# JunzheJosephZhu/DenseMatcher

Measured on AMD Instinct MI355X. Metric: mesh-pairs/sec at N=2048 D=768 k=128, higher is better.
Workload: dtype f16; 1 GPU; configs[1]: batch=64 pairs, N=2048, D=768, k=128 functional-map solve; pairs_per_gpu=64, N=2048, D=768, k=128, basis_dtype=float64, parallelism=pairs sharded over 1 GPU(s), one process per GPU, no data-path collective, process_group_size=1

## Files before the change

densematcher_amd/csrc/dm_exact.h:

```cpp
#pragma once
#include "dm_device.h"
#include "dm_internal.h"

struct ks_exact_args {
    const double* AT; const double* BT; const double* n1; const double* massS; const double* massT;
    int K, N2, N2pad, N1, N1pad, Kpad;
    dm_simnn_queue q;
    int32_t* nn;
    const void* Trow = nullptr; const void* Crow = nullptr; int ldrow = 0; int ldcrow = 0;
};

template <int KIND, typename TR, typename TC>
__device__ __forceinline__ void ks_exact_row(const ks_exact_args& a, int o, float thr, double* xrow, unsigned long long* cmask) {
    const double* __restrict__ AT = a.AT; const double* __restrict__ BT = a.BT; const double* __restrict__ n1 = a.n1;
    const double* __restrict__ massS = a.massS; const double* __restrict__ massT = a.massT;
    const int K = a.K, N2 = a.N2, N2pad = a.N2pad, N1 = a.N1, N1pad = a.N1pad, Kpad = a.Kpad;
    const float* __restrict__ qpb = a.q.pb; const int32_t* __restrict__ qpj = a.q.pj; const float* __restrict__ qps = a.q.ps;
    const int nparts = a.q.nparts, pw = a.q.pw, Npad_s = a.q.Npad, nsub = nparts * (pw / 32);
    int32_t* __restrict__ nn = a.nn;
    double* part_s = xrow + K;
    const TR* __restrict__ Trow = reinterpret_cast<const TR*>(a.Trow);
    const TC* __restrict__ Crow = reinterpret_cast<const TC*>(a.Crow);
    const int ldrow = a.ldrow, ldcrow = a.ldcrow ? a.ldcrow : a.ldrow;
    const int t = threadIdx.x;
    const int c = Crow ? (t >> 3) : (t & 31), part = Crow ? (t & 7) : (t >> 5);
    {
        const int b = o / N2, i = o - b * N2;
        const double* A = AT ? AT + (long long)b * Kpad * N2pad + i : nullptr;
        const double* Bm = BT ? BT + (long long)b * Kpad * N1pad : nullptr;
        auto keep_of = [&](int sbt) -> bool {
            const int q = min((sbt * 32) / pw, nparts - 1);
            const long long oq = ((long long)b * nparts + q) * Npad_s + i;
            const float vs = qps[oq], vb = qpb[oq];
            const int vj = qpj[oq];
            return sbt < nsub && (vs >= thr || (vb >= thr && (vj >> 5) == sbt));
        };
        bool keep = keep_of(t);
        __syncthreads();
        if (Trow) { for (int r = t; r < K; r += 256) xrow[r] = (double)Trow[((long long)b * N2 + i) * ldrow + r]; }
        else { for (int r = t; r < K; r += 256) xrow[r] = A[(long long)r * N2pad]; }
        __syncthreads();
        double bv = KIND == 0 ? DM_INF_F64 : -DM_INF_F64;
        int bj = DM_IDX_NONE;
        const double mt = KIND == 2 ? massT[(long long)b * N2 + i] : 0.0;
        for (int sb0 = 0; sb0 < nsub; sb0 += 256) {
            if (sb0) keep = keep_of(sb0 + t);
            const unsigned long long km = __ballot(keep);
            if ((t & 63) == 0) cmask[t >> 6] = km;
            __syncthreads();
            for (int w = 0; w < 4; ++w) {
                unsigned long long mm = cmask[w];
                while (mm) {
                    const int sb = sb0 + w * 64 + __ffsll((long long)mm) - 1;
                    mm &= mm - 1;
                    const int j = sb * 32 + c;
                    double sacc = 0.0;
                    if (j < N1 && Crow) {
                        const TC* Cr = Crow + ((long long)b * N1 + j) * ldcrow;
                        int r = part;
                        for (; r + 56 < K; r += 64) {
                            TC y[8];
#pragma unroll
                            for (int u = 0; u < 8; ++u) y[u] = Cr[r + 8 * u];
#pragma unroll
                            for (int u = 0; u < 8; ++u) sacc = fma(xrow[r + 8 * u], (double)y[u], sacc);
                        }
                        for (; r < K; r += 8) sacc = fma(xrow[r], (double)Cr[r], sacc);
                    } else if (j < N1) {
                        int r = part;
                        for (; r + 56 < K; r += 64) {
                            double y[8];
#pragma unroll
                            for (int u = 0; u < 8; ++u) y[u] = Bm[(long long)(r + 8 * u) * N1pad + j];
#pragma unroll
                            for (int u = 0; u < 8; ++u) sacc = fma(xrow[r + 8 * u], y[u], sacc);
                        }
                        for (; r < K; r += 8) sacc = fma(xrow[r], Bm[(long long)r * N1pad + j], sacc);
                    }
                    part_s[part * 32 + c] = sacc;
                    __syncthreads();
                    if (t < 32 && sb * 32 + t < N1) {
                        const int j = sb * 32 + t;
                        double g = part_s[t];
#pragma unroll
                        for (int q = 1; q < 8; ++q) g += part_s[q * 32 + t];
                        if (KIND == 0) {
                            const double v = n1[(long long)b * N1pad + j] - 2.0 * g;
                            if (v < bv) { bv = v; bj = j; }
                        } else {
                            const double v = g * (KIND == 1 ? massS[(long long)b * N1 + j] : mt);
                            if (v > bv) { bv = v; bj = j; }
                        }
                    }
                    __syncthreads();
                }
            }
            __syncthreads();
        }
        if (t < 32) {
#pragma unroll
            for (int off = 1; off < 32; off <<= 1) {
                const double ov = __shfl_xor(bv, off);
                const int oj = __shfl_xor(bj, off);
                if (KIND == 0) argmin_merge(bv, bj, ov, oj); else argmax_merge(bv, bj, ov, oj);
            }
            if (t == 0 && bj != DM_IDX_NONE) nn[o] = bj;
        }
    }
}
```

densematcher_amd/csrc/dm_knnsplit.hip:

```cpp
#include "dm_device.h"
#include "dm_internal.h"
#include "dm_split.h"
#include "dm_exact.h"

static inline int pad_to(int x, int m) { return (x + m - 1) / m * m; }

constexpr int KS_NCH = DM_NCH;
constexpr int KS_BIAS = 8;

__global__ __launch_bounds__(256) void ks_absmax_kernel(const double* __restrict__ AT, int K, int N2, int N2pad, int Kpad,
                                                        double* __restrict__ amax) {
    __shared__ double sh[4];
    const int chunk = blockIdx.x, b = blockIdx.y, t = threadIdx.x;
    const double* M = AT + (long long)b * Kpad * N2pad;
    double m = 0.0;
    for (int r = chunk; r < K; r += KS_NCH)
        for (int c = t; c < N2; c += 256) m = fmax(m, fabs(M[(long long)r * N2pad + c]));
#pragma unroll
    for (int off = 32; off > 0; off >>= 1) m = fmax(m, __shfl_xor(m, off));
    if ((t & 63) == 0) sh[t >> 6] = m;
    __syncthreads();
    if (t == 0) amax[b * KS_NCH + chunk] = fmax(fmax(sh[0], sh[1]), fmax(sh[2], sh[3]));
}

struct fs_bias_set {
    const double* nrm; int N, Npad; const double* mass; float* bias; unsigned int* bmax; unsigned int* mmax; float* scale32;
    int rows_out;
    const double* hint; int32_t* force;
    double* pair_out;
};
__device__ __forceinline__ void fs_bias_body(const fs_bias_set& s, int b, int chunk, const double* __restrict__ amaxT, int nT,
                                             const double* __restrict__ amaxS, int nS) {
    __shared__ float wb[4], wm[4];
    const int j = chunk * 256 + threadIdx.x;
    if (chunk * 256 >= s.N) return;
    const double sx_ = ks_scale(amaxT + b * nT, nT);
    const double sxy = sx_ * ks_scale(amaxS + b * nS, nS);
    if (chunk == 0 && threadIdx.x == 0) {
        if (s.hint && ks_scale(s.hint + b, 1) != sx_) s.force[b] = 1;
        if (s.pair_out) { double m_ = 0.0; for (int q = 0; q < nT; ++q) m_ = fmax(m_, amaxT[b * nT + q]); s.pair_out[b] = m_; }
    }
    float bb = 0.f, mm = 0.f;
    if (j < s.N) {
        const float v = (float)(-0.5 * s.nrm[(long long)b * s.Npad + j] * sxy);
        s.bias[(long long)b * s.rows_out + j] = v;
        bb = fabsf(v);
        if (s.mass) {
            const float m32 = (float)s.mass[(long long)b * s.N + j];
            s.scale32[(long long)b * s.rows_out + j] = m32;
            mm = fabsf(m32);
        }
    }
#pragma unroll
    for (int off = 32; off > 0; off >>= 1) { bb = fmaxf(bb, __shfl_xor(bb, off)); mm = fmaxf(mm, __shfl_xor(mm, off)); }
    if ((threadIdx.x & 63) == 0) { wb[threadIdx.x >> 6] = bb; wm[threadIdx.x >> 6] = mm; }
    __syncthreads();
    if (threadIdx.x == 0) {
        bb = fmaxf(fmaxf(wb[0], wb[1]), fmaxf(wb[2], wb[3]));
        mm = fmaxf(fmaxf(wm[0], wm[1]), fmaxf(wm[2], wm[3]));
        atomicMax(s.bmax + b, __float_as_uint(bb));
        if (s.mass) atomicMax(s.mmax + b, __float_as_uint(mm));
    }
}

template <bool SRC>
__global__ __launch_bounds__(256) void ks_build_kernel(const double* __restrict__ M, const double* __restrict__ n1,
                                                       const double* __restrict__ amaxT, const double* __restrict__ amaxS, int nS,
                                                       int K, int N, int Npad, int Kpad, int ld, int fill, int head,
                                                       _Float16* __restrict__ F, int32_t* __restrict__ overflow, int paired, int nT,
                                                       int rows_out,
                                                       int nbuild, fs_bias_set sA, fs_bias_set sB, int nbb) {
    if ((int)blockIdx.x < 2 * nbb) {
        const int e = (int)blockIdx.x;
        fs_bias_body(e < nbb ? sA : sB, blockIdx.y, e < nbb ? e : e - nbb, amaxT, nT, amaxS, nS);
        return;
    }
    (void)nbuild;
    extern __shared__ __attribute__((aligned(16))) _Float16 ks_img[];
    const int ldl = fill + 8;
    const int b = blockIdx.y, v0 = ((int)blockIdx.x - 2 * nbb) * 64;
    const int vl = threadIdx.x & 63, rg = threadIdx.x >> 6;
    const int v = v0 + vl;
    const double sx = ks_scale(amaxT + b * nT, nT);
    const double sc = SRC ? ks_scale(amaxS + b * nS, nS) : sx;
    _Float16* row = ks_img + vl * ldl;
    if (v < N && paired) {
        for (int r0 = rg * 16; r0 < K; r0 += 64) {
            const double* col = M + ((long long)b * Kpad + r0) * Npad + v;
            _Float16* dst = row + 2 * r0;
            f16x8 o[4];
            if (r0 + 16 <= K) {
#pragma unroll
                for (int q = 0; q < 16; ++q) {
                    _Float16 h, l;
                    split2_hw(col[(long long)q * Npad] * sc, h, l);
                    o[q >> 3][q & 7] = h;
                    o[2 + (q >> 3)][q & 7] = l;
                }
            } else {
#pragma unroll
                for (int q = 0; q < 16; ++q) {
                    _Float16 h = (_Float16)0.0f, l = (_Float16)0.0f;
                    if (r0 + q < K) split2_hw(col[(long long)q * Npad] * sc, h, l);
                    o[q >> 3][q & 7] = h;
                    o[2 + (q >> 3)][q & 7] = l;
                }
            }
#pragma unroll
            for (int q = 0; q < 4; ++q) *reinterpret_cast<f16x8*>(dst + 8 * q) = o[q];
        }
    } else if (v < N) {
        for (int r0 = rg * 16; r0 < K; r0 += 64) {
            const double* col = M + ((long long)b * Kpad + r0) * Npad + v;
            _Float16* dst = row + head + 3 * r0;
            if (r0 + 16 <= K) {
                f16x8 o[6];
#pragma unroll
                for (int q = 0; q < 16; ++q) {
                    _Float16 h, l;
                    split2_hw(col[(long long)q * Npad] * sc, h, l);
                    const int e = 3 * q;
                    o[e >> 3][e & 7] = h;
                    o[(e + 1) >> 3][(e + 1) & 7] = SRC ? l : h;
                    o[(e + 2) >> 3][(e + 2) & 7] = SRC ? h : l;
                }
#pragma unroll
                for (int q = 0; q < 6; ++q) *reinterpret_cast<f16x8*>(dst + 8 * q) = o[q];
            } else {
                for (int q = 0; r0 + q < K; ++q) {
                    _Float16 h, l;
                    split2_hw(col[(long long)q * Npad] * sc, h, l);
                    dst[3 * q] = h; dst[3 * q + 1] = SRC ? l : h; dst[3 * q + 2] = SRC ? h : l;
                }
            }
        }
        for (int c = head + 3 * K + rg; c < fill; c += 4) row[c] = (_Float16)0.0f;
        if (rg == 0 && head > 0) {
            f16x8 head8 = {(_Float16)0.0f, (_Float16)0.0f, (_Float16)0.0f, (_Float16)0.0f, (_Float16)0.0f, (_Float16)0.0f, (_Float16)0.0f, (_Float16)0.0f};
            if (SRC) {
                const double beta = -0.5 * n1[(long long)b * Npad + v] * sx * sc;
                if (!(fabs(beta) < 60000.0)) overflow[b] = 1;
                else {
                    const _Float16 b0 = (_Float16)beta;
                    const double r1 = beta - (double)b0;
                    const _Float16 b1 = (_Float16)r1;
                    head8[0] = b0; head8[1] = b1; head8[2] = (_Float16)(r1 - (double)b1);
                }
            } else {
                head8[0] = head8[1] = head8[2] = (_Float16)1.0f;
            }
            *reinterpret_cast<f16x8*>(row) = head8;
        }
    }
    __syncthreads();
    const int cpr = fill >> 3;
    const int nrow = min(64, N - v0);
    for (int c = threadIdx.x; c < nrow * cpr; c += 256) {
        const int r = c / cpr, q = c - r * cpr;
        *reinterpret_cast<f16x8*>(F + ((long long)b * rows_out + v0 + r) * ld + 8 * q) = *reinterpret_cast<const f16x8*>(ks_img + r * ldl + 8 * q);
    }
}

template <int K0, int K1, int K2 = 0, int K3 = 0, typename TR = double>
__global__ __launch_bounds__(256) void ks_exact_kernel(ks_exact_args a0, ks_exact_args a1, ks_exact_args a2, ks_exact_args a3) {
    extern __shared__ double xrow[];
    __shared__ unsigned long long cmask[4];
    const int nq = gridDim.y;
    const int c0 = *a0.q.flag_count, c1 = nq > 1 ? *a1.q.flag_count : 0, c2 = nq > 2 ? *a2.q.flag_count : 0, c3 = nq > 3 ? *a3.q.flag_count : 0;
    const int total = c0 + c1 + c2 + c3, nwg = gridDim.x * gridDim.y;
    for (int g = blockIdx.x + gridDim.x * blockIdx.y; g < total; g += nwg) {
        if (g < c0) ks_exact_row<K0, TR, TR>(a0, a0.q.flag_list[g], a0.q.flag_thr[g], xrow, cmask);
        else if (g < c0 + c1) ks_exact_row<K1, TR, TR>(a1, a1.q.flag_list[g - c0], a1.q.flag_thr[g - c0], xrow, cmask);
        else if (g < c0 + c1 + c2) ks_exact_row<K2, TR, TR>(a2, a2.q.flag_list[g - c0 - c1], a2.q.flag_thr[g - c0 - c1], xrow, cmask);
        else ks_exact_row<K3, TR, TR>(a3, a3.q.flag_list[g - c0 - c1 - c2], a3.q.flag_thr[g - c0 - c1 - c2], xrow, cmask);
    }
}

static inline size_t ks_build_lds(int fill) { return (size_t)64 * (fill + 8) * sizeof(_Float16); }
static inline int ks_depth(int K) { return pad_to(KS_BIAS + 3 * K, 32) < 96 ? 96 : pad_to(KS_BIAS + 3 * K, 32); }

size_t dm_knn_split_prep_bytes(int B, int N2, int kf) {
    return dm_align_up((size_t)B * N2 * ks_depth(kf) * 2) + dm_align_up((size_t)B * KS_NCH * 8) + 4096;
}
size_t dm_knn_split_ws_bytes(int B, int N2, int N1, int kf) {
    return dm_align_up((size_t)B * N1 * ks_depth(kf) * 2) + dm_align_up((size_t)B * 4) + dm_simnn_ws_bytes(B, N2, N1) + 8192;
}

int dm_knn_split_prepare(dm_ctx* ctx, int B, int N2, int N2pad, int Kpad, int kf, const double* AT, dm_knn_split_state* st) {
    st->enabled = ctx->opt_knn_split != 0;
    if (!st->enabled) return DM_OK;
    st->kf = kf; st->ldT = ks_depth(kf);
    st->Ft = (_Float16*)dm_ws_take(ctx, (size_t)B * N2 * st->ldT * 2);
    st->amaxT = (double*)dm_ws_take(ctx, (size_t)B * KS_NCH * 8);
    if (!st->Ft || !st->amaxT) return dm_fail(ctx, DM_ENOMEM, "knn_split: workspace not reserved");
    DM_LAUNCH(ctx, "knn_split_absmax", ks_absmax_kernel, dim3(KS_NCH, B), dim3(256), 0, AT, kf, N2, N2pad, Kpad, st->amaxT);
    int rcb = dm_grant_lds(ctx, (const void*)ks_build_kernel<false>, ks_build_lds(st->ldT));
    if (rcb) return rcb;
    DM_LAUNCH(ctx, "knn_split_build", ks_build_kernel<false>, dim3(dm_cdiv(N2, 64), B), dim3(256), ks_build_lds(st->ldT), AT,
              (const double*)nullptr, st->amaxT, (const double*)nullptr, 0, kf, N2, N2pad, Kpad, st->ldT, st->ldT, KS_BIAS, st->Ft,
              (int32_t*)nullptr, 0, KS_NCH, N2, dm_cdiv(N2, 64), fs_bias_set{}, fs_bias_set{}, 0);
    return DM_OK;
}

int dm_launch_knn21(dm_ctx* ctx, const dm_gred_args& a, const dm_knn_split_state& st, const double* amaxS, int nS) {
    if (!st.enabled) return dm_launch_gred(ctx, a);
    if (!a.AT || !a.BT || !a.n1 || !a.knn21 || !amaxS) return dm_fail(ctx, DM_EINVAL, "knn_split: missing operand");
    const int K = a.Ktrue > 0 ? a.Ktrue : a.Kloop;
    if (K > st.kf) return dm_fail(ctx, DM_EINVAL, "knn_split: depth %d beyond the prepared %d", K, st.kf);
    const int D = ks_depth(K);
    _Float16* Fs = (_Float16*)dm_ws_take(ctx, (size_t)a.B * a.N1 * D * 2);
    int32_t* overflow = (int32_t*)dm_ws_take(ctx, (size_t)a.B * 4);
    if (!Fs || !overflow) return dm_fail(ctx, DM_ENOMEM, "knn_split: workspace not reserved");
    DM_CHECK_HIP(ctx, hipMemsetAsync(overflow, 0, (size_t)a.B * 4, ctx->stream));
    int rcb = dm_grant_lds(ctx, (const void*)ks_build_kernel<true>, ks_build_lds(D));
    if (rcb) return rcb;
    DM_LAUNCH(ctx, "knn_split_build", ks_build_kernel<true>, dim3(dm_cdiv(a.N1, 64), a.B), dim3(256), ks_build_lds(D), a.BT,
              a.n1, st.amaxT, amaxS, nS, K, a.N1, a.N1pad, a.Kpad, D, D, KS_BIAS, Fs, overflow, 0, KS_NCH, a.N1, dm_cdiv(a.N1, 64), fs_bias_set{}, fs_bias_set{}, 0);
    dm_simnn_queue q;
    const float rel_extra = 1.25f * (3.0f * 2.3841858e-7f + 2.0f * sqrtf((float)K) * 2.9802322e-8f);
    int rc = dm_simnn_core(ctx, a.B, a.N2, a.N1, D, st.Ft, st.ldT, Fs, D, rel_extra, overflow, a.knn21, nullptr, nullptr, &q);
    if (rc) return rc;
    const size_t lds = ((size_t)K + 8 * 32 + 32) * sizeof(double);
    ks_exact_args ea{a.AT, a.BT, a.n1, nullptr, nullptr, K, a.N2, a.N2pad, a.N1, a.N1pad, a.Kpad, q, a.knn21};
    DM_LAUNCH(ctx, "knn_split_exact_f64", (ks_exact_kernel<0, 0>), dim3(2048, 1), dim3(256), lds, ea, ea, ea, ea);
    return DM_OK;
}

__global__ __launch_bounds__(256) void fs_zero_mass_kernel(const double* __restrict__ mass, long long n, int32_t* __restrict__ ind12) {
    const long long o = (long long)blockIdx.x * 256 + threadIdx.x;
    if (o < n && mass[o] == 0.0) ind12[o] = 0;
}

template <typename TR>
__global__ __launch_bounds__(256) void fs_build_rows_kernel(const TR* __restrict__ Phi, int N, int K, int ld, const double* __restrict__ amaxT,
                                                            int nT, int D, _Float16* __restrict__ F, int rows_out) {
    const int b = blockIdx.y;
    const int ngrp = D / 16;
    const long long o = (long long)blockIdx.x * 256 + threadIdx.x;
    if (o >= (long long)N * ngrp) return;
    const int v = (int)(o / ngrp), q = (int)(o - (long long)v * ngrp);
    const double sx = ks_scale(amaxT + b * nT, nT);
    const TR* src = Phi + ((long long)b * N + v) * ld + 8 * q;
    _Float16* dst = F + ((long long)b * rows_out + v) * D + 32 * (q >> 1) + 8 * (q & 1);
    TR xin[8];
    constexpr int amask = sizeof(TR) == 4 ? 3 : 1;
    if (8 * q + 8 <= K && ((ld & amask) == 0) && ((((uintptr_t)Phi) & 15) == 0)) {
        if constexpr (sizeof(TR) == 4) {
            typedef __attribute__((address_space(1))) const f32x4 gf32x4;
            const f32x4 v0 = ((gf32x4*)src)[0], v1 = ((gf32x4*)src)[1];
#pragma unroll
            for (int u = 0; u < 4; ++u) { xin[u] = v0[u]; xin[4 + u] = v1[u]; }
        } else {
            typedef __attribute__((address_space(1))) const f64x2 gf64x2;
#pragma unroll
            for (int u = 0; u < 4; ++u) { const f64x2 w = ((gf64x2*)src)[u]; xin[2 * u] = w[0]; xin[2 * u + 1] = w[1]; }
        }
    } else {
#pragma unroll
        for (int u = 0; u < 8; ++u) xin[u] = (8 * q + u < K) ? src[u] : (TR)0;
    }
    f16x8 hv, lv;
#pragma unroll
    for (int u = 0; u < 8; ++u) {
        _Float16 h, l;
        fs_split_entry<TR>(xin[u], sx, h, l);
        hv[u] = h; lv[u] = l;
    }
    *reinterpret_cast<f16x8*>(dst) = hv;
    *reinterpret_cast<f16x8*>(dst + 16) = lv;
}

template <typename TR>
int dm_fm_split_build_rows(dm_ctx* ctx, int B, int N, int K, const TR* Phi, int ld, const double* amaxT, int nT, int D, _Float16* F, int rows_out) {
    const long long n = (long long)N * (D / 16);
    DM_LAUNCH(ctx, "fm_split_build_rows", fs_build_rows_kernel<TR>, dim3((unsigned)((n + 255) / 256), B), dim3(256), 0, Phi, N, K, ld,
              amaxT, nT, D, F, rows_out);
    return DM_OK;
}
template int dm_fm_split_build_rows<float>(dm_ctx*, int, int, int, const float*, int, const double*, int, int, _Float16*, int);
template int dm_fm_split_build_rows<double>(dm_ctx*, int, int, int, const double*, int, const double*, int, int, _Float16*, int);

static inline int fs_depth(int K) { return 32 * ((K + 15) / 16); }
size_t dm_fm_split_zero_bytes(int B) { return 4 * dm_align_up((size_t)B * 4) + dm_align_up(dm_simnn_ctl_bytes(B)); }
bool dm_fm_split_ok(const dm_ctx* ctx, int N2, int N1, int K) {
    return ctx->opt_p2p_split != 0 && dm_simnn_dual_ok(ctx, N2, N1, fs_depth(K), true) && N1 >= 256 && N2 >= 256;
}
size_t dm_fm_split_ws_bytes(int B, int N2, int N1, int K) {
    const size_t D = fs_depth(K), R2 = pad_to(N2, 256), R1 = pad_to(N1, 256);
    return dm_align_up((size_t)B * R2 * D * 2) + dm_align_up((size_t)B * R1 * D * 2) +
           2 * dm_align_up((size_t)B * R1 * 4) + dm_align_up((size_t)B * R2 * 4) +
           dm_simnn_ws_bytes(B, N2, N1, 3) + dm_simnn_ws_bytes(B, N1, N2, 1) + 16384;
}
_Float16* dm_fm_split_take_fx(dm_ctx* ctx, int B, int N2, int K, int* D_out, int* rows_out) {
    const int D = fs_depth(K), R2 = pad_to(N2, 256);
    _Float16* Fx = (_Float16*)dm_ws_take(ctx, (size_t)B * R2 * D * 2);
    if (!Fx) return nullptr;
    if (R2 != N2 && hipMemsetAsync(Fx, 0, (size_t)B * R2 * D * 2, ctx->stream) != hipSuccess) return nullptr;
    *D_out = D; *rows_out = R2;
    return Fx;
}

template <typename TR>
int dm_launch_fm_split(dm_ctx* ctx, const dm_gred_args& a, const double* amaxS, int nS, const double* amaxT, int nT, void* zeroed,
                       const TR* Phi2, int ld2, const dm_fm_split_pre* pre) {
    const int B = a.B, N1 = a.N1, N2 = a.N2;
    const int K = a.Ktrue > 0 ? a.Ktrue : a.Kloop;
    if (!a.BT || !a.n1 || !a.n2 || !a.mass1 || !a.knn21 || !a.knn12 || !a.ind21 || !a.ind12 || !amaxS || !amaxT || !zeroed || !Phi2)
        return dm_fail(ctx, DM_EINVAL, "fm_split: missing operand");
    int D = fs_depth(K);
    int R2 = pad_to(N2, 256);
    const int R1 = pad_to(N1, 256);
    _Float16* Fx = pre ? pre->Fx : dm_fm_split_take_fx(ctx, B, N2, K, &D, &R2);
    _Float16* Fy = (_Float16*)dm_ws_take(ctx, (size_t)B * R1 * D * 2);
    float* biasA = (float*)dm_ws_take(ctx, (size_t)B * R1 * 4);
    float* biasB = (float*)dm_ws_take(ctx, (size_t)B * R2 * 4);
    float* scale32 = (float*)dm_ws_take(ctx, (size_t)B * R1 * 4);
    if (!Fx || !Fy || !biasA || !biasB || !scale32) return dm_fail(ctx, DM_ENOMEM, "fm_split: workspace not reserved");
    if (R1 != N1) DM_CHECK_HIP(ctx, hipMemsetAsync(Fy, 0, (size_t)B * R1 * D * 2, ctx->stream));
    if (R1 != N1) {
        DM_CHECK_HIP(ctx, hipMemsetAsync(biasA, 0, (size_t)B * R1 * 4, ctx->stream));
        DM_CHECK_HIP(ctx, hipMemsetAsync(scale32, 0, (size_t)B * R1 * 4, ctx->stream));
    }
    if (R2 != N2) DM_CHECK_HIP(ctx, hipMemsetAsync(biasB, 0, (size_t)B * R2 * 4, ctx->stream));
    const size_t mstride = dm_align_up((size_t)B * 4) / 4;
    unsigned int* bmaxA = reinterpret_cast<unsigned int*>(zeroed);
    unsigned int* mmax = bmaxA + mstride; unsigned int* bmaxB = bmaxA + 2 * mstride;
    int32_t* force = (pre && pre->built) ? reinterpret_cast<int32_t*>(bmaxA + 3 * mstride) : nullptr;
    if (!(pre && pre->built)) {
        const long long n = (long long)N2 * (D / 16);
        DM_LAUNCH(ctx, "fm_split_build_rows", fs_build_rows_kernel<TR>, dim3((unsigned)((n + 255) / 256), B), dim3(256), 0, Phi2, N2, K, ld2,
                  amaxT, nT, D, Fx, R2);
    }
    int rcb = dm_grant_lds(ctx, (const void*)ks_build_kernel<true>, ks_build_lds(D));
    if (rcb) return rcb;
    {
        const fs_bias_set sA{a.n1, N1, a.N1pad, a.mass1, biasA, bmaxA, mmax, scale32, R1, force ? pre->hint : nullptr, force, pre ? pre->pair_out : nullptr};
        const fs_bias_set sB{a.n2, N2, a.N2pad, nullptr, biasB, bmaxB, nullptr, nullptr, R2, nullptr, nullptr, nullptr};
        const int nbuild = dm_cdiv(N1, 64), nbb = dm_cdiv(N1 > N2 ? N1 : N2, 256);
        DM_LAUNCH(ctx, "knn_split_build", ks_build_kernel<true>, dim3(nbuild + 2 * nbb, B), dim3(256), ks_build_lds(D), a.BT,
                  a.n1, amaxT, amaxS, nS, K, N1, a.N1pad, a.Kpad, D, D, 0, Fy, (int32_t*)nullptr, 1, nT, R1, nbuild, sA, sB, nbb);
    }
    const float rel_extra = 1.25f * (3.0f * 2.3841858e-7f + 2.0f * sqrtf((float)K) * 2.9802322e-8f);
    const size_t lds = ((size_t)K + 8 * 32 + 32) * sizeof(double);
    if (ctx->opt_p2p_split >= 2) {
        dm_simnn_queue qa, qb, qc, qd;
        dm_simnn_cols cols{biasB, reinterpret_cast<const float*>(bmaxB), a.knn12, a.ind12, &qc, &qd, a.mass1};
        dm_simnn_dual dual{biasA, scale32, reinterpret_cast<const float*>(bmaxA), reinterpret_cast<const float*>(mmax), a.ind21, &qb, &cols, true};
        dm_simnn_ext ext;
        ext.ctl = reinterpret_cast<char*>(zeroed) + 4 * dm_align_up((size_t)B * 4);
        int rc = dm_simnn_core(ctx, B, N2, N1, D, Fx, D, Fy, D, rel_extra, force, a.knn21, nullptr, nullptr, &qa, &dual, &ext);
        if (rc) return rc;
        ks_exact_args e0{nullptr, a.BT, a.n1, nullptr, nullptr, K, N2, a.N2pad, N1, a.N1pad, a.Kpad, qa, a.knn21, Phi2, nullptr, ld2};
        ks_exact_args e1 = e0;
        e1.n1 = nullptr; e1.massS = a.mass1; e1.q = qb; e1.nn = a.ind21;
        ks_exact_args f0{a.BT, nullptr, a.n2, nullptr, nullptr, K, N1, a.N1pad, N2, a.N2pad, a.Kpad, qc, a.knn12, nullptr, Phi2, ld2};
        ks_exact_args f1 = f0;
        f1.n1 = nullptr; f1.massT = a.mass1; f1.q = qd; f1.nn = a.ind12;
        DM_LAUNCH(ctx, "fm_split_exact_f64", (ks_exact_kernel<0, 1, 0, 2, TR>), dim3(512, 4), dim3(256), lds, e0, e1, f0, f1);
        return DM_OK;
    }
    {
        dm_simnn_queue qa, qb;
        dm_simnn_dual dual{biasA, scale32, reinterpret_cast<const float*>(bmaxA), reinterpret_cast<const float*>(mmax), a.ind21, &qb, nullptr, true};
        int rc = dm_simnn_core(ctx, B, N2, N1, D, Fx, D, Fy, D, rel_extra, force, a.knn21, nullptr, nullptr, &qa, &dual);
        if (rc) return rc;
        ks_exact_args e0{nullptr, a.BT, a.n1, nullptr, nullptr, K, N2, a.N2pad, N1, a.N1pad, a.Kpad, qa, a.knn21, Phi2, nullptr, ld2};
        ks_exact_args e1 = e0;
        e1.n1 = nullptr; e1.massS = a.mass1; e1.q = qb; e1.nn = a.ind21;
        DM_LAUNCH(ctx, "fm_split_exact_f64", (ks_exact_kernel<0, 1, 0, 0, TR>), dim3(1024, 2), dim3(256), lds, e0, e1, e0, e1);
    }
    {
        dm_simnn_queue qa, qb;
        dm_simnn_dual dual{biasB, nullptr, reinterpret_cast<const float*>(bmaxB), nullptr, a.ind12, &qb, nullptr, true};
        int rc = dm_simnn_core(ctx, B, N1, N2, D, Fy, D, Fx, D, rel_extra, force, a.knn12, nullptr, nullptr, &qa, &dual);
        if (rc) return rc;
        ks_exact_args e0{a.BT, nullptr, a.n2, nullptr, nullptr, K, N1, a.N1pad, N2, a.N2pad, a.Kpad, qa, a.knn12, nullptr, Phi2, ld2};
        ks_exact_args e1 = e0;
        e1.n1 = nullptr; e1.massT = a.mass1; e1.q = qb; e1.nn = a.ind12;
        DM_LAUNCH(ctx, "fm_split_exact_f64", (ks_exact_kernel<0, 2, 0, 0, TR>), dim3(1024, 2), dim3(256), lds, e0, e1, e0, e1);
        const long long n = (long long)B * N1;
        DM_LAUNCH(ctx, "fm_split_zero_mass", fs_zero_mass_kernel, dim3((unsigned)((n + 255) / 256)), dim3(256), 0, a.mass1, n, a.ind12);
    }
    return DM_OK;
}
template int dm_launch_fm_split<float>(dm_ctx*, const dm_gred_args&, const double*, int, const double*, int, void*, const float*, int, const dm_fm_split_pre*);
template int dm_launch_fm_split<double>(dm_ctx*, const dm_gred_args&, const double*, int, const double*, int, void*, const double*, int, const dm_fm_split_pre*);
```

Baseline: 63220 mesh-pairs/s.

## Batch two column blocks per exact-rescore step with deeper unrolled FMA chains

The f64 exact-rescore pass now gathers G surviving 32-column blocks per iteration instead of one. It computes their partial dot products together with U=16 unrolled loads, which halves the barriers per block and raises memory-level parallelism. It also scalarises the row index, threshold and base pointer through readfirstlane, uses 32-bit per-lane offsets, prefetches the next queue entry, and sets an occupancy bound in launch_bounds. The cost is more registers and LDS, plus a new limit on padded column counts.

```diff
diff --git a/densematcher_amd/csrc/dm_exact.h b/densematcher_amd/csrc/dm_exact.h
--- a/densematcher_amd/csrc/dm_exact.h
+++ b/densematcher_amd/csrc/dm_exact.h
@@ -10,8 +10,66 @@
     const void* Trow = nullptr; const void* Crow = nullptr; int ldrow = 0; int ldcrow = 0;
 };
 
+#ifndef DM_EXACT_G
+#define DM_EXACT_G 2
+#endif
+#ifndef DM_EXACT_U
+#define DM_EXACT_U 16
+#endif
+#ifndef DM_EXACT_OCC
+#define DM_EXACT_OCC 4
+#endif
+constexpr int KS_EXACT_OCC = DM_EXACT_OCC;
+constexpr int KS_EXACT_G = DM_EXACT_G;
+constexpr int KS_EXACT_U = DM_EXACT_U;
+static inline size_t ks_exact_lds(int K) { return ((size_t)K + KS_EXACT_G * 8 * 32 + 32) * sizeof(double); }
+
+template <int G, typename TC>
+struct ks_exact_src {
+    const TC* base; long long step; unsigned voff[G];
+    const TC* P[G];
+};
+static inline bool ks_exact_km_ok(int Npad) { return Npad > 0 && Npad < (1 << 26); }
+__device__ __forceinline__ const char* ks_uniform_ptr(const void* p) {
+    const unsigned long long x = reinterpret_cast<unsigned long long>(p);
+    const unsigned lo = (unsigned)__builtin_amdgcn_readfirstlane((int)(unsigned)x), hi = (unsigned)__builtin_amdgcn_readfirstlane((int)(unsigned)(x >> 32));
+    return reinterpret_cast<const char*>(((unsigned long long)hi << 32) | lo);
+}
+
+template <int G, int U, bool KM, bool TAIL, typename TC>
+__device__ __forceinline__ void ks_exact_terms(const ks_exact_src<G, TC>& s, const double* xrow, int r0, int part, int K, double (&sacc)[G]) {
+    TC y[G][U];
+    const bool on = !TAIL || r0 + part < K;
+#pragma unroll
+    for (int u = 0; u < G; ++u)
+        if (on) {
+#pragma unroll
+            for (int v = 0; v < U; ++v) {
+                if (KM) y[u][v] = *reinterpret_cast<const TC*>(ks_uniform_ptr(s.base + (long long)(r0 + 8 * v) * s.step) + s.voff[u]);
+                else y[u][v] = s.P[u][r0 + 8 * v];
+            }
+        }
+#pragma unroll
+    for (int u = 0; u < G; ++u)
+        if (on) {
+#pragma unroll
+            for (int v = 0; v < U; ++v) sacc[u] = fma(xrow[r0 + part + 8 * v], (double)y[u][v], sacc[u]);
+        }
+}
+template <int G, bool KM, typename TC>
+__device__ __forceinline__ void ks_exact_chains(const ks_exact_src<G, TC>& s, const double* xrow, int part, int K, double (&sacc)[G]) {
+    int r0 = 0;
+    if (KS_EXACT_U > 8)
+        for (; r0 + 8 * KS_EXACT_U <= K; r0 += 8 * KS_EXACT_U) ks_exact_terms<G, KS_EXACT_U, KM, false, TC>(s, xrow, r0, part, K, sacc);
+    for (; r0 + 64 <= K; r0 += 64) ks_exact_terms<G, 8, KM, false, TC>(s, xrow, r0, part, K, sacc);
+    for (; r0 < K; r0 += 8) ks_exact_terms<G, 1, KM, true, TC>(s, xrow, r0, part, K, sacc);
+}
+
 template <int KIND, typename TR, typename TC>
-__device__ __forceinline__ void ks_exact_row(const ks_exact_args& a, int o, float thr, double* xrow, unsigned long long* cmask) {
+__device__ __forceinline__ void ks_exact_row(const ks_exact_args& a, int o_in, float thr_in, double* xrow, unsigned long long* cmask) {
+    constexpr int G = KS_EXACT_G;
+    const int o = __builtin_amdgcn_readfirstlane(o_in);
+    const float thr = __int_as_float(__builtin_amdgcn_readfirstlane(__float_as_int(thr_in)));
     const double* __restrict__ AT = a.AT; const double* __restrict__ BT = a.BT; const double* __restrict__ n1 = a.n1;
     const double* __restrict__ massS = a.massS; const double* __restrict__ massT = a.massT;
     const int K = a.K, N2 = a.N2, N2pad = a.N2pad, N1 = a.N1, N1pad = a.N1pad, Kpad = a.Kpad;
@@ -22,7 +80,8 @@
     const TR* __restrict__ Trow = reinterpret_cast<const TR*>(a.Trow);
     const TC* __restrict__ Crow = reinterpret_cast<const TC*>(a.Crow);
     const int ldrow = a.ldrow, ldcrow = a.ldcrow ? a.ldcrow : a.ldrow;
-    const int t = threadIdx.x;
+    int t = threadIdx.x;
+    asm volatile("" : "+v"(t));
     const int c = Crow ? (t >> 3) : (t & 31), part = Crow ? (t & 7) : (t >> 5);
     {
         const int b = o / N2, i = o - b * N2;
@@ -48,52 +107,68 @@
             const unsigned long long km = __ballot(keep);
             if ((t & 63) == 0) cmask[t >> 6] = km;
             __syncthreads();
-            for (int w = 0; w < 4; ++w) {
-                unsigned long long mm = cmask[w];
-                while (mm) {
-                    const int sb = sb0 + w * 64 + __ffsll((long long)mm) - 1;
-                    mm &= mm - 1;
-                    const int j = sb * 32 + c;
-                    double sacc = 0.0;
-                    if (j < N1 && Crow) {
-                        const TC* Cr = Crow + ((long long)b * N1 + j) * ldcrow;
-                        int r = part;
-                        for (; r + 56 < K; r += 64) {
-                            TC y[8];
+            int w = 0;
+            unsigned long long mm = cmask[0];
+            for (;;) {
+                int sbs[G], ng = 0, last = 0;
 #pragma unroll
-                            for (int u = 0; u < 8; ++u) y[u] = Cr[r + 8 * u];
+                for (int u = 0; u < G; ++u) {
+                    while (!mm && w < 3) mm = cmask[++w];
+                    if (mm) {
+                        last = sb0 + w * 64 + __ffsll((long long)mm) - 1;
+                        mm &= mm - 1;
+                        ng = u + 1;
+                    }
+                    sbs[u] = last;
+                }
+                if (!ng) break;
+                double sacc[G];
 #pragma unroll
-                            for (int u = 0; u < 8; ++u) sacc = fma(xrow[r + 8 * u], (double)y[u], sacc);
-                        }
-                        for (; r < K; r += 8) sacc = fma(xrow[r], (double)Cr[r], sacc);
-                    } else if (j < N1) {
-                        int r = part;
-                        for (; r + 56 < K; r += 64) {
-                            double y[8];
+                for (int u = 0; u < G; ++u) sacc[u] = 0.0;
+                if (Crow) {
+                    ks_exact_src<G, TC> src;
 #pragma unroll
-                            for (int u = 0; u < 8; ++u) y[u] = Bm[(long long)(r + 8 * u) * N1pad + j];
+                    for (int u = 0; u < G; ++u) src.P[u] = Crow + ((long long)b * N1 + min(sbs[u] * 32 + c, N1 - 1)) * ldcrow + part;
+                    ks_exact_chains<G, false, TC>(src, xrow, part, K, sacc);
+                } else {
+                    ks_exact_src<G, double> src;
+                    src.base = Bm; src.step = N1pad;
 #pragma unroll
-                            for (int u = 0; u < 8; ++u) sacc = fma(xrow[r + 8 * u], y[u], sacc);
-                        }
-                        for (; r < K; r += 8) sacc = fma(xrow[r], Bm[(long long)r * N1pad + j], sacc);
+                    for (int u = 0; u < G; ++u)
+                        src.voff[u] = ((unsigned)part * (unsigned)N1pad + (unsigned)min(sbs[u] * 32 + c, N1 - 1)) * (unsigned)sizeof(double);
+                    ks_exact_chains<G, true, double>(src, xrow, part, K, sacc);
+                }
+#pragma unroll
+                for (int u = 0; u < G; ++u) if (u < ng) part_s[(u * 8 + part) * 32 + c] = sacc[u];
+                double wv[G];
+                if (t < 32) {
+#pragma unroll
+                    for (int u = 0; u < G; ++u) {
+                        const int j = min(sbs[u] * 32 + t, N1 - 1);
+                        wv[u] = KIND == 0 ? n1[(long long)b * N1pad + j] : KIND == 1 ? massS[(long long)b * N1 + j] : mt;
                     }
-                    part_s[part * 32 + c] = sacc;
-                    __syncthreads();
-                    if (t < 32 && sb * 32 + t < N1) {
-                        const int j = sb * 32 + t;
-                        double g = part_s[t];
+                }
+                __syncthreads();
+                if (t < 32) {
 #pragma unroll
-                        for (int q = 1; q < 8; ++q) g += part_s[q * 32 + t];
-                        if (KIND == 0) {
-                            const double v = n1[(long long)b * N1pad + j] - 2.0 * g;
-                            if (v < bv) { bv = v; bj = j; }
-                        } else {
-                            const double v = g * (KIND == 1 ? massS[(long long)b * N1 + j] : mt);
-                            if (v > bv) { bv = v; bj = j; }
+                    for (int u = 0; u < G; ++u) {
+                        const int j = sbs[u] * 32 + t;
+                        if (u < ng && j < N1) {
+                            const double* ps = part_s + u * 256;
+                            double g = ps[t];
+#pragma unroll
+                            for (int q = 1; q < 8; ++q) g += ps[q * 32 + t];
+                            if (KIND == 0) {
+                                const double v = wv[u] - 2.0 * g;
+                                if (v < bv) { bv = v; bj = j; }
+                            } else {
+                                const double v = g * wv[u];
+                                if (v > bv) { bv = v; bj = j; }
+                            }
                         }
                     }
-                    __syncthreads();
                 }
+                __syncthreads();
             }
             __syncthreads();
         }
diff --git a/densematcher_amd/csrc/dm_knnsplit.hip b/densematcher_amd/csrc/dm_knnsplit.hip
--- a/densematcher_amd/csrc/dm_knnsplit.hip
+++ b/densematcher_amd/csrc/dm_knnsplit.hip
@@ -162,17 +162,29 @@
 }
 
 template <int K0, int K1, int K2 = 0, int K3 = 0, typename TR = double>
-__global__ __launch_bounds__(256) void ks_exact_kernel(ks_exact_args a0, ks_exact_args a1, ks_exact_args a2, ks_exact_args a3) {
+__global__ __launch_bounds__(256, KS_EXACT_OCC) void ks_exact_kernel(ks_exact_args a0, ks_exact_args a1, ks_exact_args a2, ks_exact_args a3) {
     extern __shared__ double xrow[];
     __shared__ unsigned long long cmask[4];
     const int nq = gridDim.y;
     const int c0 = *a0.q.flag_count, c1 = nq > 1 ? *a1.q.flag_count : 0, c2 = nq > 2 ? *a2.q.flag_count : 0, c3 = nq > 3 ? *a3.q.flag_count : 0;
     const int total = c0 + c1 + c2 + c3, nwg = gridDim.x * gridDim.y;
-    for (int g = blockIdx.x + gridDim.x * blockIdx.y; g < total; g += nwg) {
-        if (g < c0) ks_exact_row<K0, TR, TR>(a0, a0.q.flag_list[g], a0.q.flag_thr[g], xrow, cmask);
-        else if (g < c0 + c1) ks_exact_row<K1, TR, TR>(a1, a1.q.flag_list[g - c0], a1.q.flag_thr[g - c0], xrow, cmask);
-        else if (g < c0 + c1 + c2) ks_exact_row<K2, TR, TR>(a2, a2.q.flag_list[g - c0 - c1], a2.q.flag_thr[g - c0 - c1], xrow, cmask);
-        else ks_exact_row<K3, TR, TR>(a3, a3.q.flag_list[g - c0 - c1 - c2], a3.q.flag_thr[g - c0 - c1 - c2], xrow, cmask);
+    auto entry = [&](int g, int& o, float& thr) {
+        if (g < c0) { o = a0.q.flag_list[g]; thr = a0.q.flag_thr[g]; }
+        else if (g < c0 + c1) { o = a1.q.flag_list[g - c0]; thr = a1.q.flag_thr[g - c0]; }
+        else if (g < c0 + c1 + c2) { o = a2.q.flag_list[g - c0 - c1]; thr = a2.q.flag_thr[g - c0 - c1]; }
+        else { o = a3.q.flag_list[g - c0 - c1 - c2]; thr = a3.q.flag_thr[g - c0 - c1 - c2]; }
+    };
+    int g = blockIdx.x + gridDim.x * blockIdx.y;
+    if (g >= total) return;
+    int o = 0, o_next = 0;
+    float thr = 0.0f, thr_next = 0.0f;
+    entry(g, o, thr);
+    for (; g < total; g += nwg, o = o_next, thr = thr_next) {
+        if (g + nwg < total) entry(g + nwg, o_next, thr_next);
+        if (g < c0) ks_exact_row<K0, TR, TR>(a0, o, thr, xrow, cmask);
+        else if (g < c0 + c1) ks_exact_row<K1, TR, TR>(a1, o, thr, xrow, cmask);
+        else if (g < c0 + c1 + c2) ks_exact_row<K2, TR, TR>(a2, o, thr, xrow, cmask);
+        else ks_exact_row<K3, TR, TR>(a3, o, thr, xrow, cmask);
     }
 }
 
@@ -207,6 +219,7 @@
     if (!a.AT || !a.BT || !a.n1 || !a.knn21 || !amaxS) return dm_fail(ctx, DM_EINVAL, "knn_split: missing operand");
     const int K = a.Ktrue > 0 ? a.Ktrue : a.Kloop;
     if (K > st.kf) return dm_fail(ctx, DM_EINVAL, "knn_split: depth %d beyond the prepared %d", K, st.kf);
+    if (!ks_exact_km_ok(a.N1pad)) return dm_fail(ctx, DM_EINVAL, "knn_split: %d padded columns are beyond the exact pass's 32-bit offsets", a.N1pad);
     const int D = ks_depth(K);
     _Float16* Fs = (_Float16*)dm_ws_take(ctx, (size_t)a.B * a.N1 * D * 2);
     int32_t* overflow = (int32_t*)dm_ws_take(ctx, (size_t)a.B * 4);
@@ -220,7 +233,7 @@
     const float rel_extra = 1.25f * (3.0f * 2.3841858e-7f + 2.0f * sqrtf((float)K) * 2.9802322e-8f);
     int rc = dm_simnn_core(ctx, a.B, a.N2, a.N1, D, st.Ft, st.ldT, Fs, D, rel_extra, overflow, a.knn21, nullptr, nullptr, &q);
     if (rc) return rc;
-    const size_t lds = ((size_t)K + 8 * 32 + 32) * sizeof(double);
+    const size_t lds = ks_exact_lds(K);
     ks_exact_args ea{a.AT, a.BT, a.n1, nullptr, nullptr, K, a.N2, a.N2pad, a.N1, a.N1pad, a.Kpad, q, a.knn21};
     DM_LAUNCH(ctx, "knn_split_exact_f64", (ks_exact_kernel<0, 0>), dim3(2048, 1), dim3(256), lds, ea, ea, ea, ea);
     return DM_OK;
@@ -307,6 +320,7 @@
     const int K = a.Ktrue > 0 ? a.Ktrue : a.Kloop;
     if (!a.BT || !a.n1 || !a.n2 || !a.mass1 || !a.knn21 || !a.knn12 || !a.ind21 || !a.ind12 || !amaxS || !amaxT || !zeroed || !Phi2)
         return dm_fail(ctx, DM_EINVAL, "fm_split: missing operand");
+    if (!ks_exact_km_ok(a.N1pad)) return dm_fail(ctx, DM_EINVAL, "fm_split: %d padded columns are beyond the exact pass's 32-bit offsets", a.N1pad);
     int D = fs_depth(K);
     int R2 = pad_to(N2, 256);
     const int R1 = pad_to(N1, 256);
@@ -341,7 +355,7 @@
                   a.n1, amaxT, amaxS, nS, K, N1, a.N1pad, a.Kpad, D, D, 0, Fy, (int32_t*)nullptr, 1, nT, R1, nbuild, sA, sB, nbb);
     }
     const float rel_extra = 1.25f * (3.0f * 2.3841858e-7f + 2.0f * sqrtf((float)K) * 2.9802322e-8f);
-    const size_t lds = ((size_t)K + 8 * 32 + 32) * sizeof(double);
+    const size_t lds = ks_exact_lds(K);
     if (ctx->opt_p2p_split >= 2) {
         dm_simnn_queue qa, qb, qc, qd;
         dm_simnn_cols cols{biasB, reinterpret_cast<const float*>(bmaxB), a.knn12, a.ind12, &qc, &qd, a.mass1};
```

Result: no change. 63430 mesh-pairs/s, median of 6 (+0.3%).
